# AdamCodd/local-hyperDB

Measured on AMD Instinct MI355X. Metric: queries/sec, N=10M d=384 fp16 top-100 (single-query stream; p50 latency alongside), higher is better.
Workload: dtype f16; 1 GPU; N=10000000 d=384 fp16 Q=1 cosine_similarity top-100, row-sharded x1; rows_per_gpu=10000000, accumulate=f32, exchange=none

## Files before the change

local-hyperdb_amd/csrc/hdb_api.hip:

```cpp
#include "hdb_common.h"
#include "hdb_quant.h"
#include "hdb_ws.h"
#include "hdb_plan.h"
#include "../../include/hyperdb_hip.h"
#include <string>
#include <cmath>
#include <cstring>
#include <cstdio>
#include <algorithm>
#include <vector>
#include <chrono>
#include <atomic>

static thread_local std::string g_err;
static int fail(int code, const std::string& msg) { g_err = msg; return code; }
#define HIP_TRY(expr)                                                                              \
    do {                                                                                           \
        hipError_t e_ = (expr);                                                                    \
        if (e_ != hipSuccess)                                                                      \
            return fail(HDB_ERR_HIP, std::string(#expr) + ": " + hipGetErrorString(e_));           \
    } while (0)
#define LAUNCH_TRY(expr)                                                                           \
    do {                                                                                           \
        int e_ = (expr);                                                                           \
// ... 697 lines not shown
    int rc = quant_ws_lay(ix, w, nq, (nq == 1 && ix->pnib) ? p.pl_cap : 0, mflavour);
    if (rc) return rc;
    const uint32_t pl_cap = p.pl_cap;
    uint32_t* pl_cnt = use_pl ? reinterpret_cast<uint32_t*>(ix->qstat) + 1 : nullptr;
    const size_t crow = (size_t)nq * HDB_CAND_CAP;
    const int nsub = p.nsub;
    rc = quant_query_prep(ix, (const float*)dev_Q, nq, w, mflavour, ix->qstat, nsub ? w.cnt : nullptr, pl_cnt, st);
    if (rc) return rc;
    QuantArgs a; quant_base_args(ix, a, w.qcodes, w.qaux, w.qinv, metric, nq);
    a.ntiles = sp.s_tiles; a.tile_stride = sp.s_stride; a.scores = w.sbuf; a.ld = sp.ld_s;
    a.wmax = w.wmax; a.nsub = nsub; a.thr_out = w.thr;
    LAUNCH_TRY(hdb_launch_quant_scan(&a, 0, (int)ix->opt.max_blocks, st));
    if (!nsub) LAUNCH_TRY(hdb_launch_sample_thr(w.sbuf, sp.s_rows, sp.ld_s, nq, m, w.thr, w.cnt, nullptr, st));
    a.ntiles = (n + 15) / 16; a.tile_stride = 1; a.scores = nullptr; a.ld = 0;
    a.thr = w.thr; a.cnt = w.cnt; a.cand = w.cand; a.cap = HDB_CAND_CAP;
    prof_begin(ix, st);
    if (use_pl) {
        a.pl_nib = ix->pnib; a.pl_bit = ix->pbit; a.pl_rec = ix->prec; a.pl_units = ix->pU;
        a.pl_list = w.pl_list; a.pl_cnt = pl_cnt; a.pl_cap = pl_cap;
        LAUNCH_TRY(hdb_launch_quant_plane_scan(&a, 0, (int)ix->opt.max_blocks, st));
        a.nsub = 0; a.wmax = nullptr;
        LAUNCH_TRY(hdb_launch_quant_scan_one(&a, 1, (int)ix->opt.max_blocks, st));
    } else {
        LAUNCH_TRY(hdb_launch_quant_scan(&a, 1, (int)ix->opt.max_blocks, st));
    }
    prof_end(ix, st);
    if (mflavour) {
        const bool has_bias = ix->bias != nullptr || ix->mask != nullptr;
        LAUNCH_TRY(hdb_launch_quant_cgather(ix->V, ix->d * 2, ix->inv_norm, ix->bias, ix->mask, w.cand, w.cnt, HDB_CAND_CAP, nq, w.G,
                                            metric == HDB_COSINE ? w.ginv : nullptr, has_bias ? w.gbias : nullptr, st));
        ScanArgs s; memset(&s, 0, sizeof(s));
        s.V = w.G; s.n = (int64_t)crow; s.d = ix->d; s.Q = dev_Q; s.metric = metric; s.inv_norm = w.ginv; s.qinv = w.qinv;
        s.bias = has_bias ? w.gbias : nullptr; s.mask = nullptr; s.nq = nq;
        s.tile_stride = 1; s.ntiles = (int64_t)crow / hdb_mfma_tile_rows(ix->dtype, ix->d); s.cap = HDB_CAND_CAP;
        s.scores = w.gsc; s.ld = (int64_t)crow;
        LAUNCH_TRY(hdb_launch_mfma_scan(&s, ix->dtype, 0, nq, w.q16, w.ginv, w.qsq, w.qscl, (int)ix->opt.max_blocks, (int)ix->opt.mfma_variant, st, nullptr));
    } else {
        LAUNCH_TRY(hdb_launch_quant_rescore(ix->V, ix->d, ix->dtype, (const float*)dev_Q, nq, metric, ix->inv_norm, w.qinv, ix->bias, ix->mask,
                                            w.cand, w.cnt, HDB_CAND_CAP, st));
    }
    LAUNCH_TRY(hdb_launch_quant_finalize(w.cand, w.cnt, HDB_CAND_CAP, nq, (uint32_t)k, kk, ix->row_base, dev_idx, dev_score, dev_status, w.qnan,
                                         w.qaux, w.thr, ix->qstat, mflavour ? w.cand : nullptr, w.gsc, (int64_t)crow, st));
    return HDB_OK;
}

// ... 711 lines not shown
```

local-hyperdb_amd/csrc/hdb_launch.h:

```cpp
#pragma once
#include <stddef.h>
#include <stdint.h>

struct ScanArgs;
struct FusedArgs;
struct BatchArgs;
struct BitsArgs;
struct QuantArgs;

#define HDB_ANYD_DECL(name) int name(const ScanArgs* args, int dpad, int mode, int nq_launch, const void* q, const float* sqnorm, \
                                     const float* qsq, const float* qscl, int blocks, void* stream)
#define HDB_GEOM_DECL(name) int name(const ScanArgs* args, int mode, int nq_launch, const void* q16, const float* sqnorm, \
                                     const float* qsq, const float* qscl, int blocks, int variant, void* stream, const BatchArgs* f)

extern "C" {
int hdb_launch_scan(const ScanArgs* args, int dtype, int mode, int nq_launch, int max_blocks, void* stream);
int hdb_launch_rownorm(const void* V, int64_t n, int d, int dtype, float* inv_norm, float* sqnorm, int* nan_flag, void* stream);
int hdb_launch_qprep(const void* Q, int nq, int d, bool f64, float* qinv, float* qsq, int* qnan, void* q16, float* qscl, void* stream);
int hdb_launch_qprep2(const void* Q, int nq, int d, bool f64, float* qinv, float* qsq, int* qnan, void* q16, float* qscl,
                      float* thr_init, uint32_t* cnt_init, uint32_t* qbits, int W, void* stream);
int hdb_launch_signpack(const void* V, int64_t n, int d, int dtype, int64_t row0, uint32_t* bits, void* stream);
int hdb_launch_qsign(const void* Q, int nq, int d, bool f64, int W, uint32_t* qbits, void* stream);
int hdb_launch_hamming(const ScanArgs* args, int mode, int nq_launch, const uint32_t* bits, int64_t npad, int W,
                       const uint32_t* qbits, void* stream);
// ... 69 lines not shown
int hdb_launch_quant_rows(const void* V, int64_t n, int d, int dtype, int P, int8_t* codes, float* aux, int* nan_flag, double gamma,
                          void* stream);
int hdb_launch_quant_gather(const int8_t* codes, const float* aux, const int64_t* rows, int64_t m, int P, int8_t* codes_out,
                            float* aux_out, void* stream);
int hdb_launch_quant_qprep(const float* Q, int nq, int d, int P, int8_t* qcodes, float* qaux, int* stat, uint32_t* pl_cnt, void* stream);
int hdb_launch_quant_qprep_m(const float* Q, int nq, int d, int P, float* qinv, float* qsq, int* qnan, void* q16, float* qscl,
                             int8_t* qcodes, float* qaux, int* stat, uint32_t* cnt_init, uint32_t* pl_cnt, void* stream);
int hdb_launch_quant_plane_rows(const int8_t* codes, const float* aux, int64_t row0, int64_t m, int d, int P, uint8_t* nib, uint32_t* bitw,
                                float* rec, void* stream);
int hdb_launch_quant_plane_scan(const QuantArgs* args, int dbg, int max_blocks, void* stream);
int hdb_launch_quant_scan(const QuantArgs* args, int mode, int max_blocks, void* stream);
int hdb_launch_quant_scan_one(const QuantArgs* args, int mode, int max_blocks, void* stream);
int hdb_launch_quant_rescore(const void* V, int d, int dtype, const float* Q, int nq, int metric, const float* inv_norm,
                             const float* qinv, const float* bias, const uint8_t* mask, unsigned long long* cand,
                             const uint32_t* cnt, uint32_t cap, void* stream);
int hdb_launch_quant_cgather(const void* V, int row_bytes, const float* inv_norm, const float* bias, const uint8_t* mask,
                             const unsigned long long* cand, const uint32_t* cnt, uint32_t cap, int nq, void* G, float* ginv, float* gbias,
                             void* stream);
int hdb_launch_quant_finalize(const unsigned long long* cand, const uint32_t* cnt, uint32_t cap, int nq, uint32_t k, uint32_t kk,
                              int64_t row_base, int64_t* idx_out, float* score_out, int32_t* status, const int* qnan,
                              const float* qaux, const float* thr, int* stat, unsigned long long* cand_rw, const float* sc, int64_t ld,
                              void* stream);

int hdb_launch_qb_scan(const QuantArgs* args, int mode, float* wstat, int64_t wld, int max_blocks, void* stream);
int hdb_launch_qb_thr(const float* vals, int64_t n, int64_t ld, int nq, uint32_t m, float* thr, void* stream);
int hdb_launch_qb_rescore(const void* V, int d, const void* q16, const float* qscl, const float* qinv, const float* inv_norm,
                          const float* bias, const uint8_t* mask, int metric, unsigned long long* cand, const uint32_t* cnt,
                          uint32_t cap, int nq, void* stream);
}
```

local-hyperdb_amd/csrc/hdb_quant.h:

```cpp
#pragma once
#include <stdint.h>

#define HDB_QROW_S 0
#define HDB_QROW_E 1
#define HDB_QROW_T 2
#define HDB_QQ_S 0
#define HDB_QQ_N 1
#define HDB_QQ_D 2
#define HDB_QQ_SQ 3
#define HDB_QQ_BAD 4
#define HDB_QQ_CN 5
#define HDB_QQ_CS 6
#define HDB_QQ_WORDS 8

struct QuantArgs {
    const int8_t* codes;
    int64_t n;
    int32_t d;
    int32_t P;
    const float* aux;
    const float* sqnorm;
    const float* inv_norm;
    const int8_t* qcodes;
    const float* qaux;
    const float* qinv;
    const float* bias;
    const uint8_t* mask;
    int32_t metric;
    int32_t nq;
    float gamma;
    int64_t ntiles;
    int64_t tile_stride;
    float* scores; int64_t ld;
    const float* thr; uint32_t* cnt; unsigned long long* cand; uint32_t cap;
    uint32_t* wmax; int32_t nsub; float* thr_out;
    const uint8_t* pl_nib; const uint32_t* pl_bit; const float* pl_rec; int32_t pl_units;
    uint32_t* pl_list; uint32_t* pl_cnt; uint32_t pl_cap;
    float* dbg;
};
#define HDB_QUANT_NSUB_MAX 4096
```

local-hyperdb_amd/csrc/hdb_quant.hip:

```cpp
#include "hdb_common.h"
#include "hdb_quant.h"
#include "hdb_finalize.h"
#include "../../include/hyperdb_hip.h"

__device__ __forceinline__ float hq_up(double x) {
    x = x * (1.0 + 0x1p-40);
    float f = (float)x;
    if ((double)f < x) f = nextafterf(f, INFINITY);
    return f;
}

__device__ __forceinline__ float hq_f(__half v) { return __half2float(v); }
__device__ __forceinline__ float hq_f(float v) { return v; }

template <typename T> struct HqElem;
template <> struct HqElem<__half> { static constexpr int EPC = 8; };
template <> struct HqElem<float> { static constexpr int EPC = 4; };

__device__ __forceinline__ void hq_unpack(const uint4& raw, float (&x)[8], __half*) {
    const __half2* h = reinterpret_cast<const __half2*>(&raw);
#pragma unroll
    for (int i = 0; i < 4; ++i) { float2 f = __half22float2(h[i]); x[2 * i] = f.x; x[2 * i + 1] = f.y; }
}
__device__ __forceinline__ void hq_unpack(const uint4& raw, float (&x)[4], float*) {
// ... 206 lines not shown
    case 2: return __builtin_amdgcn_update_dpp(0, x, HDB_DPP_XOR2, 0xF, 0xF, false);
    default: return __builtin_amdgcn_update_dpp(0, x, HDB_DPP_XOR1, 0xF, 0xF, false);
    }
}
__device__ __forceinline__ int hq_rows4_sum(int a0, int a1, int a2, int a3, int l16) {
    const bool b3 = (l16 & 8) != 0, b2 = (l16 & 4) != 0;
    const int v01 = (b3 ? a1 : a0) + hq_dpp_i(b3 ? a0 : a1, 0);
    const int v23 = (b3 ? a3 : a2) + hq_dpp_i(b3 ? a2 : a3, 0);
    int w = (b2 ? v23 : v01) + hq_dpp_i(b2 ? v01 : v23, 1);
    w += hq_dpp_i(w, 2);
    w += hq_dpp_i(w, 3);
    return w;
}

template <int NQ>
__device__ __forceinline__ void hq_fold_thr(const QuantArgs& a, float (&q_thr)[NQ]) {
    __shared__ uint32_t s_top[4 * 16];
    __shared__ float s_thr[NQ];
    const int ln = threadIdx.x & 63, wv = threadIdx.x >> 6;
    for (int q = 0; q < NQ; ++q) {
        uint32_t c[HDB_QUANT_NSUB_MAX / 256];
#pragma unroll
        for (int j = 0; j < HDB_QUANT_NSUB_MAX / 256; ++j) {
            const int e = (int)threadIdx.x + 256 * j;
            c[j] = e < a.nsub ? a.wmax[(int64_t)q * a.nsub + e] : 0u;
        }
        for (int r = 0; r < 16; ++r) {
            uint32_t lm = 0u;
#pragma unroll
            for (int j = 0; j < HDB_QUANT_NSUB_MAX / 256; ++j) lm = max(lm, c[j]);
            uint32_t wm = lm;
#pragma unroll
            for (int o = 32; o > 0; o >>= 1) wm = max(wm, (uint32_t)__shfl_xor((int)wm, o, 64));
            const unsigned long long who = __ballot(lm == wm);
            if (ln == (int)__ffsll((long long)who) - 1) {
                bool gone = false;
#pragma unroll
                for (int j = 0; j < HDB_QUANT_NSUB_MAX / 256; ++j)
                    if (!gone && c[j] == wm) { c[j] = 0u; gone = true; }
            }
// ... 9 lines not shown
                for (int o = 32; o > 0; o >>= 1) wm = max(wm, (uint32_t)__shfl_xor((int)wm, o, 64));
                const unsigned long long who = __ballot(v == wm);
                if (ln == (int)__ffsll((long long)who) - 1) v = 0u;
                kth = wm;
            }
            if (ln == 0) {
                const float t = kth == 0u ? -INFINITY : hdb_key2f(kth);
                s_thr[q] = t;
                if (blockIdx.x == 0) a.thr_out[q] = t;
            }
        }
        __syncthreads();
    }
#pragma unroll
    for (int q = 0; q < NQ; ++q) q_thr[q] = s_thr[q];
}

template <int MODE, int NQ, int NJ, bool LIST = false>
__global__ __launch_bounds__(256) void hdb_quant_scan_kernel(QuantArgs a) {
    extern __shared__ __attribute__((aligned(16))) char smem[];
    int4* qs = reinterpret_cast<int4*>(smem);
    __shared__ HqStage stage;
    const int nch = a.P >> 4;
    static_assert(!LIST || (MODE == 1 && NQ == 1), "the list flavour is pass 2 of a one-query call");
    if (MODE == 1 && threadIdx.x < 4) stage.cnt[threadIdx.x] = 0u;
    for (int i = threadIdx.x; i < NQ * nch; i += 256) qs[i] = reinterpret_cast<const int4*>(a.qcodes)[i];
    float q_s[NQ], q_n[NQ], q_d[NQ], q_sq[NQ], q_inv[NQ], q_thr[NQ];
    bool q_bad[NQ];
#pragma unroll
    for (int q = 0; q < NQ; ++q) {
        const float* o = a.qaux + (int64_t)q * HDB_QQ_WORDS;
        q_s[q] = o[HDB_QQ_S]; q_n[q] = o[HDB_QQ_N]; q_d[q] = o[HDB_QQ_D]; q_sq[q] = o[HDB_QQ_SQ]; q_bad[q] = o[HDB_QQ_BAD] != 0.f;
        q_inv[q] = a.metric == HDB_COSINE ? a.qinv[q] : 1.f;
        q_thr[q] = (MODE == 1 && a.nsub == 0) ? a.thr[q] : 0.f;
    }
    __syncthreads();
    if (MODE == 1 && a.nsub > 0) hq_fold_thr<NQ>(a, q_thr);

    const int lane = threadIdx.x & 63, wave = threadIdx.x >> 6;
    const int g = lane >> 4, l16 = lane & 15;
    const int nj = NJ > 0 ? NJ : (nch + 15) >> 4;
    constexpr int G = NJ > 0 ? NJ : 2;
    const float absmin = 0x1p-100f * (float)(a.d + 8);
    const float g2 = 2.f * a.gamma;
    typedef unsigned int u32x4 __attribute__((ext_vector_type(4)));
    uint32_t wbest[NQ];
#pragma unroll
    for (int q = 0; q < NQ; ++q) wbest[q] = 0u;

    int64_t ntiles = a.ntiles;
    uint32_t pl_n = 0u;
    bool pl_list = false;
// ... 2 lines not shown
        pl_list = pl_n <= a.pl_cap;
        if (pl_list) ntiles = ((int64_t)pl_n + 15) >> 4;
        else if (blockIdx.x == 0 && threadIdx.x == 0) atomicAdd(&a.pl_cnt[1], 1u);
    }
    for (int64_t t = (int64_t)blockIdx.x * 4 + wave; t < ntiles; t += (int64_t)gridDim.x * 4) {
        const int64_t r0 = hdb_tile_index(t, a.tile_stride) * 16 + 4 * g;
        int64_t rr[4];
#pragma unroll
        for (int u = 0; u < 4; ++u) {
            rr[u] = r0 + u;
            if (LIST && pl_list) rr[u] = (uint64_t)(r0 + u) < (uint64_t)pl_n ? (int64_t)a.pl_list[r0 + u] : a.n;
        }
        const int8_t* p[4];
#pragma unroll
        for (int u = 0; u < 4; ++u) p[u] = a.codes + min(rr[u], a.n - 1) * (int64_t)a.P;
        int acc[4][NQ];
#pragma unroll
        for (int u = 0; u < 4; ++u)
#pragma unroll
            for (int q = 0; q < NQ; ++q) acc[u][q] = 0;
        for (int j0 = 0; j0 < nj; j0 += G) {
            uint4 raw[G][4];
#pragma unroll
            for (int j = 0; j < G; ++j) {
                const int c = l16 + 16 * (j0 + j);
                const bool live = (j0 + j) < nj && c < nch;
#pragma unroll
                for (int u = 0; u < 4; ++u) {
                    if (live) {
                        const u32x4 v = __builtin_nontemporal_load(reinterpret_cast<const u32x4*>(p[u] + (int64_t)c * 16));
// ... 11 lines not shown
#pragma unroll
                for (int q = 0; q < NQ; ++q) {
                    const int4 qv = qs[q * nch + cc];
#pragma unroll
                    for (int u = 0; u < 4; ++u) {
                        int s = acc[u][q];
                        s = __builtin_amdgcn_sdot4((int)raw[j][u].x, qv.x, s, false);
                        s = __builtin_amdgcn_sdot4((int)raw[j][u].y, qv.y, s, false);
                        s = __builtin_amdgcn_sdot4((int)raw[j][u].z, qv.z, s, false);
                        s = __builtin_amdgcn_sdot4((int)raw[j][u].w, qv.w, s, false);
                        acc[u][q] = s;
                    }
                }
            }
        }
        const int u_own = hdb_owned_row(l16);
        const int64_t row = LIST ? (u_own == 0 ? rr[0] : u_own == 1 ? rr[1] : u_own == 2 ? rr[2] : rr[3]) : r0 + u_own;
        int C[NQ];
#pragma unroll
        for (int q = 0; q < NQ; ++q) C[q] = hq_rows4_sum(acc[0][q], acc[1][q], acc[2][q], acc[3][q], l16);
        if ((l16 & 3) != 0) continue;
        const int64_t out_i = t * 16 + 4 * g + u_own;
        if (row >= a.n) {
            if (MODE == 0 && a.nsub == 0)
#pragma unroll
                for (int q = 0; q < NQ; ++q) a.scores[(int64_t)q * a.ld + out_i] = -INFINITY;
            continue;
        }
        const float s_r = a.aux[3 * row + HDB_QROW_S], e_r = a.aux[3 * row + HDB_QROW_E], t_r = a.aux[3 * row + HDB_QROW_T];
        const bool masked = a.mask && !a.mask[row];
        const float bias = a.bias ? a.bias[row] : 0.f;
        const float invn = a.metric == HDB_COSINE ? a.inv_norm[row] : 1.f;
        const float sqv = a.metric == HDB_EUCLIDEAN ? a.sqnorm[row] : 0.f;
#pragma unroll
        for (int q = 0; q < NQ; ++q) {
            float lo = -INFINITY, hi = -INFINITY;
            if (!q_bad[q] && !masked) {
                const float A = (q_s[q] * s_r) * (float)C[q];
                const float aA = fabsf(A);
                const float B = (q_n[q] * e_r + q_d[q] * t_r) * (1.f + 0x1p-10f) + aA * 0x1p-10f + absmin;
                if (a.metric == HDB_EUCLIDEAN) {
                    const float ctr = sqv + q_sq[q] - 2.f * A;
                    const float err = g2 * sqv + 2.f * B + 0x1p-10f * (sqv + q_sq[q] + 2.f * aA) + absmin;
                    const float elo = fmaxf(ctr - err, 0.f) * (1.f - g2 - 0x1p-10f);
                    const float ehi = (ctr + err) * (1.f + g2 + 0x1p-10f);
                    hi = (float)(1.f / (1.f + sqrt(elo)));
                    lo = (float)(1.f / (1.f + sqrt(ehi)));
                } else {
// ... 5 lines not shown
                hi = hi + fabsf(hi) * 0x1p-20f + 1e-30f;
                if (lo != lo) lo = -INFINITY;
                if (hi != hi) hi = INFINITY;
            }
            if (MODE == 2) {
                a.dbg[row] = hi;
            } else if (MODE == 0) {
                if (a.nsub > 0) wbest[q] = max(wbest[q], hdb_f2key(lo));
                else a.scores[(int64_t)q * a.ld + out_i] = lo;
            } else if (!masked && !q_bad[q] && hi >= q_thr[q]) {
                const unsigned long long ent = hdb_pack(hi, (uint32_t)row);
                const unsigned int lp = atomicAdd(&stage.cnt[q], 1u);
                if (lp < HQ_STAGE_CAP) stage.buf[q][lp] = ent;
                else {
                    const uint32_t pos = atomicAdd(&a.cnt[q * HDB_CNT_STRIDE], 1u);
                    if (pos < a.cap) a.cand[(int64_t)q * a.cap + pos] = ent;
                }
            }
        }
    }
    if (MODE == 0 && a.nsub > 0) {
#pragma unroll
        for (int q = 0; q < NQ; ++q) {
            uint32_t wm = wbest[q];
#pragma unroll
            for (int o = 32; o > 0; o >>= 1) wm = max(wm, (uint32_t)__shfl_xor((int)wm, o, 64));
            if (lane == 0) a.wmax[(int64_t)q * a.nsub + blockIdx.x * 4 + wave] = wm;
        }
    }
    if (MODE == 1) {
        __syncthreads();
        for (int q = 0; q < NQ; ++q) {
            const unsigned int have = min(stage.cnt[q], (unsigned int)HQ_STAGE_CAP);
            if (have == 0u) continue;
            if (threadIdx.x == 0) stage.base = atomicAdd(&a.cnt[q * HDB_CNT_STRIDE], have);
            __syncthreads();
            const unsigned int base = stage.base;
            for (unsigned int e = threadIdx.x; e < have; e += blockDim.x)
                if (base + e < a.cap) a.cand[(int64_t)q * a.cap + base + e] = stage.buf[q][e];
            __syncthreads();
        }
    }
}

__global__ __launch_bounds__(256) void hdb_quant_plane_rows_kernel(const int8_t* codes, const float* aux, int64_t row0, int64_t m, int d, int P,
                                                                   int U, uint8_t* nib, uint32_t* bitw, float* rec) {
    const int lane = threadIdx.x & 63, g = lane >> 4, l16 = lane & 15;
    const int64_t wave = ((int64_t)blockIdx.x * 256 + threadIdx.x) >> 6;
    const int64_t nwaves = ((int64_t)gridDim.x * 256) >> 6;
    for (int64_t base = wave * 4; base < m; base += nwaves * 4) {
        const int64_t r = row0 + base + g;
        const bool valid = base + g < m;
        int ss = 0;
        if (valid && l16 < U) {
// ... 17 lines not shown
                }
            }
            *reinterpret_cast<uint4*>(nib + (r * (int64_t)U + l16) * 16) = make_uint4(nw[0], nw[1], nw[2], nw[3]);
            bitw[r * (int64_t)U + l16] = bw;
        }
#pragma unroll
        for (int o = 8; o > 0; o >>= 1) ss += __shfl_xor(ss, o, 64);
        if (valid && l16 == 0) {
            const float R = sqrtf((float)ss) * (1.f + 0x1p-20f);
            *reinterpret_cast<float4*>(rec + 4 * r) = make_float4(aux[3 * r + HDB_QROW_S], aux[3 * r + HDB_QROW_E], aux[3 * r + HDB_QROW_T], R);
        }
    }
}

#define HQ_PL_STAGE 1024
template <int J, bool DBG>
__global__ __launch_bounds__(256) void hdb_quant_plane_scan_kernel(QuantArgs a) {
    extern __shared__ __attribute__((aligned(16))) char smem[];
    int4* qs = reinterpret_cast<int4*>(smem);
    __shared__ int part[4][2][64 * J];
    __shared__ uint32_t st_buf[HQ_PL_STAGE];
    __shared__ uint32_t st_cnt, st_base;
    const int U = a.pl_units, nch = a.P >> 4;
    if (threadIdx.x == 0) st_cnt = 0u;
    for (int i = threadIdx.x; i < 2 * U; i += 256) qs[i] = i < nch ? reinterpret_cast<const int4*>(a.qcodes)[i] : make_int4(0, 0, 0, 0);
    const float* qo = a.qaux;
    const float q_s = qo[HDB_QQ_S], q_n = qo[HDB_QQ_N], q_d = qo[HDB_QQ_D], q_cn = qo[HDB_QQ_CN];
    const int q_cs = (int)qo[HDB_QQ_CS];
    const bool q_bad = qo[HDB_QQ_BAD] != 0.f;
    const bool cosine = a.metric == HDB_COSINE;
    const float q_inv = cosine ? a.qinv[0] : 1.f;
    float thr1[1] = {(!DBG && a.nsub == 0) ? a.thr[0] : 0.f};
    __syncthreads();
    if (!DBG && a.nsub > 0) hq_fold_thr<1>(a, thr1);
    const float q_thr = thr1[0];

    const int lane = threadIdx.x & 63, wave = threadIdx.x >> 6;
    const int npieces = 16 * U;
    int qw[J][8];
    int prow[J];
#pragma unroll
    for (int j = 0; j < J; ++j) {
        const int f = lane + 64 * j;
        const int unit = f < npieces ? f % U : 0;
        prow[j] = f < npieces ? f / U : 16;
        const int4 x = qs[2 * unit], y = qs[2 * unit + 1];
        qw[j][0] = x.x; qw[j][1] = x.y; qw[j][2] = x.z; qw[j][3] = x.w;
        qw[j][4] = y.x; qw[j][5] = y.y; qw[j][6] = y.z; qw[j][7] = y.w;
    }
    const float absmin = 0x1p-100f * (float)(a.d + 8);
    typedef unsigned int u32x4 __attribute__((ext_vector_type(4)));
    typedef float f32x4 __attribute__((ext_vector_type(4)));
    const int64_t ntiles = a.ntiles;
    const int et = lane >> 4, er = lane & 15;

    for (int64_t t = ((int64_t)blockIdx.x * 4 + wave) * 2; t < ntiles; t += (int64_t)gridDim.x * 8) {
        u32x4 nv[2][J];
        uint32_t bv[2][J];
#pragma unroll
        for (int tt = 0; tt < 2; ++tt) {
            const int64_t rows_left = a.n - (t + tt) * 16;
            const uint8_t* nb = a.pl_nib + (t + tt) * (int64_t)npieces * 16;
            const uint32_t* bb = a.pl_bit + (t + tt) * (int64_t)npieces;
#pragma unroll
            for (int j = 0; j < J; ++j) {
                const int f = lane + 64 * j;
                if ((int64_t)prow[j] < rows_left && prow[j] < 16) {
                    nv[tt][j] = __builtin_nontemporal_load(reinterpret_cast<const u32x4*>(nb + (int64_t)f * 16));
                    bv[tt][j] = __builtin_nontemporal_load(bb + f);
                } else {
                    nv[tt][j] = u32x4{0u, 0u, 0u, 0u};
                    bv[tt][j] = 0u;
                }
            }
        }
        const int64_t row = (t + et) * 16 + er;
        const bool rvalid = lane < 32 && t + et < ntiles && row < a.n;
        f32x4 rc = f32x4{0.f, 0.f, 0.f, 0.f};
        float invn = 1.f, bias = 0.f;
        bool masked = false;
        if (rvalid) {
            rc = __builtin_nontemporal_load(reinterpret_cast<const f32x4*>(a.pl_rec) + row);
            if (cosine) invn = a.inv_norm[row];
            if (a.bias) bias = a.bias[row];
            if (a.mask) masked = !a.mask[row];
        }
        __builtin_amdgcn_sched_barrier(0);
#pragma unroll
        for (int tt = 0; tt < 2; ++tt) {
#pragma unroll
            for (int j = 0; j < J; ++j) {
                const uint32_t bw = bv[tt][j];
                const uint32_t w4[4] = {nv[tt][j].x, nv[tt][j].y, nv[tt][j].z, nv[tt][j].w};
                int s = 0;
#pragma unroll
                for (int i = 0; i < 4; ++i) {
                    const uint32_t lo = ((w4[i] << 1) & 0x1E1E1E1Eu) | ((bw >> (2 * i)) & 0x01010101u);
                    const uint32_t hi = ((w4[i] >> 3) & 0x1E1E1E1Eu) | ((bw >> (2 * i + 1)) & 0x01010101u);
                    s = __builtin_amdgcn_sdot4((int)lo, qw[j][2 * i], s, false);
                    s = __builtin_amdgcn_sdot4((int)hi, qw[j][2 * i + 1], s, false);
                }
                part[wave][tt][lane + 64 * j] = s;
            }
        }
        __builtin_amdgcn_fence(__ATOMIC_RELEASE, "wavefront");
        __builtin_amdgcn_wave_barrier();
        __builtin_amdgcn_fence(__ATOMIC_ACQUIRE, "wavefront");
        int S = 0;
        if (lane < 32)
            for (int i = 0; i < U; ++i) S += part[wave][et][er * U + i];
        __builtin_amdgcn_fence(__ATOMIC_RELEASE, "wavefront");
        __builtin_amdgcn_wave_barrier();
        if (!rvalid) continue;
        float hi5 = -INFINITY;
        const bool dead = masked || q_bad;
        if (!dead) {
            const float fc = (float)(8 * S - 124 * q_cs);
            const float Uf = q_cn * rc.w;
            float ch = fc + Uf, cl = fc - Uf;
            ch = ch + (fabsf(ch) * 0x1p-20f + 1.f);
            cl = cl - (fabsf(cl) * 0x1p-20f + 1.f);
            const float k = q_s * rc.x;
            const float A5 = k * ch, Al = k * cl;
            const float Amax = fmaxf(fabsf(A5), fabsf(Al));
            const float c0 = (q_n * rc.y + q_d * rc.z) * (1.f + 0x1p-10f);
            const float B5 = c0 + fabsf(A5) * 0x1p-10f + absmin;
            const float Bmax = c0 + Amax * 0x1p-10f + absmin;
            const float Mx = Amax + Bmax;
            float X = (A5 + B5) + (Mx * 0x1p-18f + 1e-30f);
            float mM = Mx * (1.f + 0x1p-17f);
// ... 1 lines not shown
            const float Z = mM + fabsf(bias);
            float h = X;
            if (a.bias) h += bias;
            hi5 = h + (Z * 0x1p-18f + 4e-30f);
            if (hi5 != hi5) hi5 = INFINITY;
        }
        if (DBG) {
            a.dbg[row] = hi5;
        } else if (!dead && !(hi5 < q_thr)) {
            const unsigned int lp = atomicAdd(&st_cnt, 1u);
            if (lp < HQ_PL_STAGE) st_buf[lp] = (uint32_t)row;
            else {
                const uint32_t pos = atomicAdd(&a.pl_cnt[0], 1u);
                if (pos < a.pl_cap) a.pl_list[pos] = (uint32_t)row;
            }
        }
    }
    if (!DBG) {
        __syncthreads();
        const unsigned int have = min(st_cnt, (unsigned int)HQ_PL_STAGE);
        if (have != 0u) {
            if (threadIdx.x == 0) st_base = atomicAdd(&a.pl_cnt[0], have);
            __syncthreads();
            const unsigned int base = st_base;
            for (unsigned int e = threadIdx.x; e < have; e += blockDim.x)
                if (base + e < a.pl_cap) a.pl_list[base + e] = st_buf[e];
        }
    }
}

// ... 58 lines not shown
                s = (float)(Acc(1) / (Acc(1) + sqrt(sum)));
            } else if (a.metric == HDB_COSINE) {
                s = (float)sum * a.inv_norm[row] * a.qinv[q];
            } else {
                s = (float)sum;
            }
            if (a.bias) s += a.bias[row];
            const bool masked = a.mask && !a.mask[row];
            if (masked) s = -INFINITY;
            s = hdb_canon(s);
            a.cand[(int64_t)q * a.cap + i] = hdb_pack(s, row);
        }
    }
}

__global__ __launch_bounds__(256) void hdb_quant_cgather_kernel(const char* V, int row_bytes, const float* inv_norm, const float* bias,
                                                                const uint8_t* mask, const unsigned long long* cand, const uint32_t* cnt,
                                                                uint32_t cap, char* G, float* ginv, float* gbias) {
    const int q = blockIdx.y, lane = threadIdx.x & 63, wave = threadIdx.x >> 6;
    const uint32_t total = min(cnt[q * HDB_CNT_STRIDE], cap);
    for (uint32_t i = blockIdx.x * 4 + wave; i < total; i += gridDim.x * 4) {
        const int64_t slot = (int64_t)q * cap + i;
        const uint32_t row = 0xFFFFFFFFu - (uint32_t)(cand[slot] & 0xFFFFFFFFull);
        const char* src = V + (int64_t)row * row_bytes;
        char* dst = G + slot * row_bytes;
        for (int c = lane * 16; c < row_bytes; c += 64 * 16) *reinterpret_cast<uint4*>(dst + c) = *reinterpret_cast<const uint4*>(src + c);
        if (lane == 0) {
            if (ginv) ginv[slot] = inv_norm[row];
            if (gbias) gbias[slot] = mask ? (mask[row] ? (bias ? bias[row] : 0.f) : -INFINITY) : bias[row];
        }
    }
}

__global__ __launch_bounds__(1024) void hdb_quant_finalize_kernel(const unsigned long long* cand, const uint32_t* cnt, uint32_t cap, uint32_t k,
                                                                  uint32_t kk, int64_t row_base, int64_t* idx_out, float* score_out,
                                                                  int32_t* status, const int* qnan, const float* qaux, const float* thr,
                                                                  int* stat, unsigned long long* cand_rw, const float* sc, int64_t ld) {
    extern __shared__ __attribute__((aligned(16))) unsigned long long buf[];
    const int q = blockIdx.x;
    const uint32_t total = cnt[q * HDB_CNT_STRIDE];
    if (sc) {
        const uint32_t nc = min(total, cap);
        for (uint32_t i = threadIdx.x; i < nc; i += blockDim.x) {
            const int64_t slot = (int64_t)q * cap + i;
            const uint32_t row = 0xFFFFFFFFu - (uint32_t)(cand_rw[slot] & 0xFFFFFFFFull);
            cand_rw[slot] = hdb_pack(sc[(int64_t)q * ld + slot], row);
        }
        __threadfence_block();
// ... 25 lines not shown
}

extern "C" int hdb_launch_quant_qprep(const float* Q, int nq, int d, int P, int8_t* qcodes, float* qaux, int* stat, uint32_t* pl_cnt,
                                      void* stream) {
    hipLaunchKernelGGL(hdb_quant_qprep_kernel, dim3(nq), dim3(64), 0, (hipStream_t)stream, Q, nq, d, P, qcodes, qaux, stat, pl_cnt);
    return (int)hipGetLastError();
}

extern "C" int hdb_launch_quant_qprep_m(const float* Q, int nq, int d, int P, float* qinv, float* qsq, int* qnan, void* q16, float* qscl,
                                        int8_t* qcodes, float* qaux, int* stat, uint32_t* cnt_init, uint32_t* pl_cnt, void* stream) {
    hipLaunchKernelGGL(hdb_quant_qprep_m_kernel, dim3(nq), dim3(64), 0, (hipStream_t)stream, Q, nq, d, P, qinv, qsq, qnan, (_Float16*)q16,
                       qscl, qcodes, qaux, stat, cnt_init, pl_cnt);
    return (int)hipGetLastError();
}

extern "C" int hdb_launch_quant_cgather(const void* V, int row_bytes, const float* inv_norm, const float* bias, const uint8_t* mask,
                                        const unsigned long long* cand, const uint32_t* cnt, uint32_t cap, int nq, void* G, float* ginv,
                                        float* gbias, void* stream) {
    if (row_bytes % 16 != 0 || (reinterpret_cast<uintptr_t>(V) & 15) != 0) return (int)hipErrorInvalidValue;
    hipLaunchKernelGGL(hdb_quant_cgather_kernel, dim3(256, nq), dim3(256), 0, (hipStream_t)stream, (const char*)V, row_bytes, inv_norm, bias,
                       mask, cand, cnt, cap, (char*)G, ginv, gbias);
    return (int)hipGetLastError();
}

template <int MODE, int NQ>
static void hq_launch_scan_nq(const QuantArgs& a, int blocks, size_t lds, hipStream_t st) {
    const int nch = a.P >> 4;
    const int nj = (nch + 15) >> 4;
    if (nj == 1) hipLaunchKernelGGL((hdb_quant_scan_kernel<MODE, NQ, 1>), dim3(blocks), dim3(256), lds, st, a);
    else if (nj == 2) hipLaunchKernelGGL((hdb_quant_scan_kernel<MODE, NQ, 2>), dim3(blocks), dim3(256), lds, st, a);
    else if (nj == 3) hipLaunchKernelGGL((hdb_quant_scan_kernel<MODE, NQ, 3>), dim3(blocks), dim3(256), lds, st, a);
    else hipLaunchKernelGGL((hdb_quant_scan_kernel<MODE, NQ, 0>), dim3(blocks), dim3(256), lds, st, a);
}
template <int MODE>
static void hq_launch_scan_mode(const QuantArgs& a, int blocks, size_t lds, hipStream_t st) {
    switch (a.nq) {
    case 1: hq_launch_scan_nq<MODE, 1>(a, blocks, lds, st); break;
    case 2: hq_launch_scan_nq<MODE, 2>(a, blocks, lds, st); break;
    case 3: hq_launch_scan_nq<MODE, 3>(a, blocks, lds, st); break;
    default: hq_launch_scan_nq<MODE, 4>(a, blocks, lds, st); break;
    }
}
extern "C" int hdb_launch_quant_scan(const QuantArgs* args, int mode, int max_blocks, void* stream) {
    const QuantArgs& a = *args;
    if (a.nq < 1 || a.nq > 4 || (a.P & 15) != 0) return (int)hipErrorInvalidValue;
    const size_t lds = (size_t)a.nq * a.P;
    const int blocks = hdb_quant_scan_blocks(a.ntiles, max_blocks);
    if (a.nsub != 0 && (a.nsub > HDB_QUANT_NSUB_MAX || !a.wmax || (mode == 0 ? a.nsub != 4 * blocks : !a.thr_out))) return (int)hipErrorInvalidValue;
    if (mode == 0) hq_launch_scan_mode<0>(a, blocks, lds, (hipStream_t)stream);
    else hq_launch_scan_mode<1>(a, blocks, lds, (hipStream_t)stream);
    return (int)hipGetLastError();
}

extern "C" int hdb_launch_quant_plane_rows(const int8_t* codes, const float* aux, int64_t row0, int64_t m, int d, int P, uint8_t* nib,
                                           uint32_t* bitw, float* rec, void* stream) {
    if (m <= 0) return 0;
    const int U = hdb_quant_plane_units(P);
    if (U > 16 || (P & 15) != 0) return (int)hipErrorInvalidValue;
    hipLaunchKernelGGL(hdb_quant_plane_rows_kernel, dim3(hdb_grid_for(m, 16, 8192)), dim3(256), 0, (hipStream_t)stream, codes, aux, row0, m, d,
                       P, U, nib, bitw, rec);
    return (int)hipGetLastError();
}
extern "C" int hdb_launch_quant_plane_scan(const QuantArgs* args, int dbg, int max_blocks, void* stream) {
    const QuantArgs& a = *args;
    const int U = a.pl_units;
    if (a.nq != 1 || U < 1 || U > 16 || U != hdb_quant_plane_units(a.P) || (a.metric != HDB_DOT && a.metric != HDB_COSINE)) return (int)hipErrorInvalidValue;
    if (!dbg && a.nsub != 0 && (a.nsub > HDB_QUANT_NSUB_MAX || !a.wmax || !a.thr_out)) return (int)hipErrorInvalidValue;
    const size_t lds = (size_t)U * 32;
    const int blocks = hdb_grid_for((a.ntiles + 1) / 2, 4, max_blocks > 0 ? max_blocks : 1024);
    hipStream_t st = (hipStream_t)stream;
    const int J = (U + 3) / 4;
#define HQ_PLANE(J_) do { if (dbg) hipLaunchKernelGGL((hdb_quant_plane_scan_kernel<J_, true>), dim3(blocks), dim3(256), lds, st, a); \
                          else hipLaunchKernelGGL((hdb_quant_plane_scan_kernel<J_, false>), dim3(blocks), dim3(256), lds, st, a); } while (0)
    if (J == 1) HQ_PLANE(1); else if (J == 2) HQ_PLANE(2); else if (J == 3) HQ_PLANE(3); else HQ_PLANE(4);
#undef HQ_PLANE
    return (int)hipGetLastError();
}
extern "C" int hdb_launch_quant_scan_one(const QuantArgs* args, int mode, int max_blocks, void* stream) {
    const QuantArgs& a = *args;
    if (a.nq != 1 || (a.P & 15) != 0 || a.nsub != 0 || (mode != 1 && mode != 2)) return (int)hipErrorInvalidValue;
    const size_t lds = (size_t)a.P;
    const int blocks = hdb_quant_scan_blocks(a.ntiles, max_blocks);
    const int nj = ((a.P >> 4) + 15) >> 4;
    hipStream_t st = (hipStream_t)stream;
#define HQ_ONE(NJ_) do { if (mode == 1) hipLaunchKernelGGL((hdb_quant_scan_kernel<1, 1, NJ_, true>), dim3(blocks), dim3(256), lds, st, a); \
                         else hipLaunchKernelGGL((hdb_quant_scan_kernel<2, 1, NJ_, false>), dim3(blocks), dim3(256), lds, st, a); } while (0)
    if (nj == 1) HQ_ONE(1); else if (nj == 2) HQ_ONE(2); else if (nj == 3) HQ_ONE(3); else HQ_ONE(0);
#undef HQ_ONE
    return (int)hipGetLastError();
}

extern "C" int hdb_launch_quant_rescore(const void* V, int d, int dtype, const float* Q, int nq, int metric, const float* inv_norm,
                                        const float* qinv, const float* bias, const uint8_t* mask, unsigned long long* cand,
                                        const uint32_t* cnt, uint32_t cap, void* stream) {
    hipStream_t st = (hipStream_t)stream;
// ... 34 lines not shown
```

Baseline: 1870 queries/s.

## Fuse candidate row gather into quant scan and software-pipeline plane scan loads

Removes the separate candidate-gather kernel: the quant scan now copies the fp16 row, inverse norm and bias into the gather buffer at the moment a candidate is appended. The plane scan kernel is restructured into a double-buffered loop that issues the next tile's nibble, bit and per-row loads before decoding the current tile. It also overlaps the first loads with the threshold fold and prefetches per-row aux data before the dot loop in the generic scan. The aim is to save a kernel launch plus a second pass over candidates and to hide memory latency, at the cost of more registers and scattered per-candidate copies inside the hot scan.

```diff
diff --git a/local-hyperdb_amd/csrc/hdb_api.hip b/local-hyperdb_amd/csrc/hdb_api.hip
--- a/local-hyperdb_amd/csrc/hdb_api.hip
+++ b/local-hyperdb_amd/csrc/hdb_api.hip
@@ -735,6 +735,11 @@
     if (!nsub) LAUNCH_TRY(hdb_launch_sample_thr(w.sbuf, sp.s_rows, sp.ld_s, nq, m, w.thr, w.cnt, nullptr, st));
     a.ntiles = (n + 15) / 16; a.tile_stride = 1; a.scores = nullptr; a.ld = 0;
     a.thr = w.thr; a.cnt = w.cnt; a.cand = w.cand; a.cap = HDB_CAND_CAP;
+    const bool has_bias = ix->bias != nullptr || ix->mask != nullptr;
+    if (mflavour) {
+        a.V = (const char*)ix->V; a.row_bytes = ix->d * 2; a.G = w.G;
+        a.ginv = metric == HDB_COSINE ? w.ginv : nullptr; a.gbias = has_bias ? w.gbias : nullptr;
+    }
     prof_begin(ix, st);
     if (use_pl) {
         a.pl_nib = ix->pnib; a.pl_bit = ix->pbit; a.pl_rec = ix->prec; a.pl_units = ix->pU;
@@ -747,9 +752,6 @@
     }
     prof_end(ix, st);
     if (mflavour) {
-        const bool has_bias = ix->bias != nullptr || ix->mask != nullptr;
-        LAUNCH_TRY(hdb_launch_quant_cgather(ix->V, ix->d * 2, ix->inv_norm, ix->bias, ix->mask, w.cand, w.cnt, HDB_CAND_CAP, nq, w.G,
-                                            metric == HDB_COSINE ? w.ginv : nullptr, has_bias ? w.gbias : nullptr, st));
         ScanArgs s; memset(&s, 0, sizeof(s));
         s.V = w.G; s.n = (int64_t)crow; s.d = ix->d; s.Q = dev_Q; s.metric = metric; s.inv_norm = w.ginv; s.qinv = w.qinv;
         s.bias = has_bias ? w.gbias : nullptr; s.mask = nullptr; s.nq = nq;
diff --git a/local-hyperdb_amd/csrc/hdb_launch.h b/local-hyperdb_amd/csrc/hdb_launch.h
--- a/local-hyperdb_amd/csrc/hdb_launch.h
+++ b/local-hyperdb_amd/csrc/hdb_launch.h
@@ -107,9 +107,6 @@
 int hdb_launch_quant_rescore(const void* V, int d, int dtype, const float* Q, int nq, int metric, const float* inv_norm,
                              const float* qinv, const float* bias, const uint8_t* mask, unsigned long long* cand,
                              const uint32_t* cnt, uint32_t cap, void* stream);
-int hdb_launch_quant_cgather(const void* V, int row_bytes, const float* inv_norm, const float* bias, const uint8_t* mask,
-                             const unsigned long long* cand, const uint32_t* cnt, uint32_t cap, int nq, void* G, float* ginv, float* gbias,
-                             void* stream);
 int hdb_launch_quant_finalize(const unsigned long long* cand, const uint32_t* cnt, uint32_t cap, int nq, uint32_t k, uint32_t kk,
                               int64_t row_base, int64_t* idx_out, float* score_out, int32_t* status, const int* qnan,
                               const float* qaux, const float* thr, int* stat, unsigned long long* cand_rw, const float* sc, int64_t ld,
diff --git a/local-hyperdb_amd/csrc/hdb_quant.h b/local-hyperdb_amd/csrc/hdb_quant.h
--- a/local-hyperdb_amd/csrc/hdb_quant.h
+++ b/local-hyperdb_amd/csrc/hdb_quant.h
@@ -37,5 +37,6 @@
     const uint8_t* pl_nib; const uint32_t* pl_bit; const float* pl_rec; int32_t pl_units;
     uint32_t* pl_list; uint32_t* pl_cnt; uint32_t pl_cap;
     float* dbg;
+    const char* V; int32_t row_bytes; char* G; float* ginv; float* gbias;
 };
 #define HDB_QUANT_NSUB_MAX 4096
diff --git a/local-hyperdb_amd/csrc/hdb_quant.hip b/local-hyperdb_amd/csrc/hdb_quant.hip
--- a/local-hyperdb_amd/csrc/hdb_quant.hip
+++ b/local-hyperdb_amd/csrc/hdb_quant.hip
@@ -244,16 +244,26 @@
 }
 
 template <int NQ>
-__device__ __forceinline__ void hq_fold_thr(const QuantArgs& a, float (&q_thr)[NQ]) {
+__device__ __forceinline__ void hq_fold_keys(const QuantArgs& a, int q, uint32_t (&c)[HDB_QUANT_NSUB_MAX / 256]) {
+#pragma unroll
+    for (int j = 0; j < HDB_QUANT_NSUB_MAX / 256; ++j) {
+        const int e = (int)threadIdx.x + 256 * j;
+        const uint32_t v = a.wmax[(int64_t)q * a.nsub + min(e, a.nsub - 1)];
+        c[j] = e < a.nsub ? v : 0u;
+    }
+}
+template <int NQ>
+__device__ __forceinline__ void hq_fold_thr(const QuantArgs& a, float (&q_thr)[NQ], const uint32_t (&k0)[HDB_QUANT_NSUB_MAX / 256]) {
     __shared__ uint32_t s_top[4 * 16];
     __shared__ float s_thr[NQ];
     const int ln = threadIdx.x & 63, wv = threadIdx.x >> 6;
     for (int q = 0; q < NQ; ++q) {
         uint32_t c[HDB_QUANT_NSUB_MAX / 256];
-#pragma unroll
-        for (int j = 0; j < HDB_QUANT_NSUB_MAX / 256; ++j) {
-            const int e = (int)threadIdx.x + 256 * j;
-            c[j] = e < a.nsub ? a.wmax[(int64_t)q * a.nsub + e] : 0u;
+        if (q == 0) {
+#pragma unroll
+            for (int j = 0; j < HDB_QUANT_NSUB_MAX / 256; ++j) c[j] = k0[j];
+        } else {
+            hq_fold_keys<NQ>(a, q, c);
         }
         for (int r = 0; r < 16; ++r) {
             uint32_t lm = 0u;
@@ -293,6 +303,16 @@
     }
 #pragma unroll
     for (int q = 0; q < NQ; ++q) q_thr[q] = s_thr[q];
+}
+
+__device__ __forceinline__ void hq_gather_row(const QuantArgs& a, int64_t slot, uint32_t row, int l0, int nl) {
+    const char* src = a.V + (int64_t)row * a.row_bytes;
+    char* dst = a.G + slot * a.row_bytes;
+    for (int c = l0 * 16; c < a.row_bytes; c += nl * 16) *reinterpret_cast<uint4*>(dst + c) = *reinterpret_cast<const uint4*>(src + c);
+    if (l0 == 0) {
+        if (a.ginv) a.ginv[slot] = a.inv_norm[row];
+        if (a.gbias) a.gbias[slot] = a.mask ? (a.mask[row] ? (a.bias ? a.bias[row] : 0.f) : -INFINITY) : a.bias[row];
+    }
 }
 
 template <int MODE, int NQ, int NJ, bool LIST = false>
@@ -314,7 +334,11 @@
         q_thr[q] = (MODE == 1 && a.nsub == 0) ? a.thr[q] : 0.f;
     }
     __syncthreads();
-    if (MODE == 1 && a.nsub > 0) hq_fold_thr<NQ>(a, q_thr);
+    if (MODE == 1 && a.nsub > 0) {
+        uint32_t keys[HDB_QUANT_NSUB_MAX / 256];
+        hq_fold_keys<NQ>(a, 0, keys);
+        hq_fold_thr<NQ>(a, q_thr, keys);
+    }
 
     const int lane = threadIdx.x & 63, wave = threadIdx.x >> 6;
     const int g = lane >> 4, l16 = lane & 15;
@@ -347,6 +371,17 @@
         const int8_t* p[4];
 #pragma unroll
         for (int u = 0; u < 4; ++u) p[u] = a.codes + min(rr[u], a.n - 1) * (int64_t)a.P;
+        const int u_own = hdb_owned_row(l16);
+        const int64_t row = LIST ? (u_own == 0 ? rr[0] : u_own == 1 ? rr[1] : u_own == 2 ? rr[2] : rr[3]) : r0 + u_own;
+        float s_r = 0.f, e_r = 0.f, t_r = 0.f, bias = 0.f, invn = 1.f, sqv = 0.f;
+        bool masked = false;
+        if ((l16 & 3) == 0 && row < a.n) {
+            s_r = a.aux[3 * row + HDB_QROW_S]; e_r = a.aux[3 * row + HDB_QROW_E]; t_r = a.aux[3 * row + HDB_QROW_T];
+            if (a.mask) masked = !a.mask[row];
+            if (a.bias) bias = a.bias[row];
+            if (a.metric == HDB_COSINE) invn = a.inv_norm[row];
+            if (a.metric == HDB_EUCLIDEAN) sqv = a.sqnorm[row];
+        }
         int acc[4][NQ];
 #pragma unroll
         for (int u = 0; u < 4; ++u)
@@ -388,8 +423,6 @@
                 }
             }
         }
-        const int u_own = hdb_owned_row(l16);
-        const int64_t row = LIST ? (u_own == 0 ? rr[0] : u_own == 1 ? rr[1] : u_own == 2 ? rr[2] : rr[3]) : r0 + u_own;
         int C[NQ];
 #pragma unroll
         for (int q = 0; q < NQ; ++q) C[q] = hq_rows4_sum(acc[0][q], acc[1][q], acc[2][q], acc[3][q], l16);
@@ -401,11 +434,6 @@
                 for (int q = 0; q < NQ; ++q) a.scores[(int64_t)q * a.ld + out_i] = -INFINITY;
             continue;
         }
-        const float s_r = a.aux[3 * row + HDB_QROW_S], e_r = a.aux[3 * row + HDB_QROW_E], t_r = a.aux[3 * row + HDB_QROW_T];
-        const bool masked = a.mask && !a.mask[row];
-        const float bias = a.bias ? a.bias[row] : 0.f;
-        const float invn = a.metric == HDB_COSINE ? a.inv_norm[row] : 1.f;
-        const float sqv = a.metric == HDB_EUCLIDEAN ? a.sqnorm[row] : 0.f;
 #pragma unroll
         for (int q = 0; q < NQ; ++q) {
             float lo = -INFINITY, hi = -INFINITY;
@@ -441,7 +469,10 @@
                 if (lp < HQ_STAGE_CAP) stage.buf[q][lp] = ent;
                 else {
                     const uint32_t pos = atomicAdd(&a.cnt[q * HDB_CNT_STRIDE], 1u);
-                    if (pos < a.cap) a.cand[(int64_t)q * a.cap + pos] = ent;
+                    if (pos < a.cap) {
+                        a.cand[(int64_t)q * a.cap + pos] = ent;
+                        if (a.G) hq_gather_row(a, (int64_t)q * a.cap + pos, (uint32_t)row, 0, 1);
+                    }
                 }
             }
         }
@@ -465,6 +496,10 @@
             const unsigned int base = stage.base;
             for (unsigned int e = threadIdx.x; e < have; e += blockDim.x)
                 if (base + e < a.cap) a.cand[(int64_t)q * a.cap + base + e] = stage.buf[q][e];
+            if (a.G)
+                for (unsigned int e = wave; e < have; e += 4)
+                    if (base + e < a.cap)
+                        hq_gather_row(a, (int64_t)q * a.cap + base + e, 0xFFFFFFFFu - (uint32_t)(stage.buf[q][e] & 0xFFFFFFFFull), lane, 64);
             __syncthreads();
         }
     }
@@ -512,8 +547,46 @@
 }
 
 #define HQ_PL_STAGE 1024
+#ifndef HQ_PL_BLOCKS
+#define HQ_PL_BLOCKS 1024
+#endif
+typedef unsigned int hq_u32x4 __attribute__((ext_vector_type(4)));
+typedef float hq_f32x4 __attribute__((ext_vector_type(4)));
+template <int J>
+struct HqPlStep {
+    hq_u32x4 nv[2][J];
+    uint32_t bv[2][J];
+    hq_f32x4 rc;
+    float invn, bias;
+    uint8_t mask;
+};
+template <int J>
+__device__ __forceinline__ void hq_pl_issue(const QuantArgs& a, int64_t t, int lane, int npieces, const int (&prow)[J], bool cosine,
+                                            HqPlStep<J>& s) {
+#pragma unroll
+    for (int tt = 0; tt < 2; ++tt) {
+        const int64_t rows_left = a.n - (t + tt) * 16;
+        const int64_t f0 = (t + tt) * (int64_t)npieces + lane;
+#pragma unroll
+        for (int j = 0; j < J; ++j) {
+            const int64_t f = ((int64_t)prow[j] < rows_left && prow[j] < 16) ? f0 + 64 * j : 0;
+            s.nv[tt][j] = __builtin_nontemporal_load(reinterpret_cast<const hq_u32x4*>(a.pl_nib) + f);
+            s.bv[tt][j] = __builtin_nontemporal_load(a.pl_bit + f);
+        }
+    }
+    const int64_t row = (t + (lane >> 4)) * 16 + (lane & 15);
+    const int64_t rowc = (lane < 32 && row < a.n) ? row : 0;
+    const float* invp = cosine ? a.inv_norm : a.pl_rec;
+    const float* biasp = a.bias ? a.bias : a.pl_rec;
+    const uint8_t* maskp = a.mask ? a.mask : reinterpret_cast<const uint8_t*>(a.pl_rec);
+    s.rc = __builtin_nontemporal_load(reinterpret_cast<const hq_f32x4*>(a.pl_rec) + rowc);
+    s.invn = invp[rowc];
+    s.bias = biasp[rowc];
+    s.mask = maskp[rowc];
+}
+
 template <int J, bool DBG>
-__global__ __launch_bounds__(256) void hdb_quant_plane_scan_kernel(QuantArgs a) {
+__global__ __launch_bounds__(256, 4) void hdb_quant_plane_scan_kernel(QuantArgs a) {
     extern __shared__ __attribute__((aligned(16))) char smem[];
     int4* qs = reinterpret_cast<int4*>(smem);
     __shared__ int part[4][2][64 * J];
@@ -529,76 +602,50 @@
     const bool cosine = a.metric == HDB_COSINE;
     const float q_inv = cosine ? a.qinv[0] : 1.f;
     float thr1[1] = {(!DBG && a.nsub == 0) ? a.thr[0] : 0.f};
-    __syncthreads();
-    if (!DBG && a.nsub > 0) hq_fold_thr<1>(a, thr1);
-    const float q_thr = thr1[0];
+    uint32_t keys[HDB_QUANT_NSUB_MAX / 256] = {};
+    if (!DBG && a.nsub > 0) hq_fold_keys<1>(a, 0, keys);
 
     const int lane = threadIdx.x & 63, wave = threadIdx.x >> 6;
     const int npieces = 16 * U;
-    int qw[J][8];
     int prow[J];
 #pragma unroll
-    for (int j = 0; j < J; ++j) {
-        const int f = lane + 64 * j;
-        const int unit = f < npieces ? f % U : 0;
-        prow[j] = f < npieces ? f / U : 16;
-        const int4 x = qs[2 * unit], y = qs[2 * unit + 1];
-        qw[j][0] = x.x; qw[j][1] = x.y; qw[j][2] = x.z; qw[j][3] = x.w;
-        qw[j][4] = y.x; qw[j][5] = y.y; qw[j][6] = y.z; qw[j][7] = y.w;
-    }
+    for (int j = 0; j < J; ++j) prow[j] = lane + 64 * j < npieces ? (lane + 64 * j) / U : 16;
+    const int64_t ntiles = a.ntiles;
+    const int64_t tstep = (int64_t)gridDim.x * 8;
+    int64_t t = ((int64_t)blockIdx.x * 4 + wave) * 2;
+    HqPlStep<J> s0, s1;
+    hq_pl_issue<J>(a, t, lane, npieces, prow, cosine, s0);
+    __builtin_amdgcn_sched_barrier(0);
+
+    __syncthreads();
+    if (!DBG && a.nsub > 0) hq_fold_thr<1>(a, thr1, keys);
+    const float q_thr = thr1[0];
+    int qoff[J];
+#pragma unroll
+    for (int j = 0; j < J; ++j) qoff[j] = lane + 64 * j < npieces ? 2 * ((lane + 64 * j) % U) : 0;
     const float absmin = 0x1p-100f * (float)(a.d + 8);
-    typedef unsigned int u32x4 __attribute__((ext_vector_type(4)));
-    typedef float f32x4 __attribute__((ext_vector_type(4)));
-    const int64_t ntiles = a.ntiles;
     const int et = lane >> 4, er = lane & 15;
 
-    for (int64_t t = ((int64_t)blockIdx.x * 4 + wave) * 2; t < ntiles; t += (int64_t)gridDim.x * 8) {
-        u32x4 nv[2][J];
-        uint32_t bv[2][J];
-#pragma unroll
-        for (int tt = 0; tt < 2; ++tt) {
-            const int64_t rows_left = a.n - (t + tt) * 16;
-            const uint8_t* nb = a.pl_nib + (t + tt) * (int64_t)npieces * 16;
-            const uint32_t* bb = a.pl_bit + (t + tt) * (int64_t)npieces;
-#pragma unroll
-            for (int j = 0; j < J; ++j) {
-                const int f = lane + 64 * j;
-                if ((int64_t)prow[j] < rows_left && prow[j] < 16) {
-                    nv[tt][j] = __builtin_nontemporal_load(reinterpret_cast<const u32x4*>(nb + (int64_t)f * 16));
-                    bv[tt][j] = __builtin_nontemporal_load(bb + f);
-                } else {
-                    nv[tt][j] = u32x4{0u, 0u, 0u, 0u};
-                    bv[tt][j] = 0u;
-                }
-            }
-        }
-        const int64_t row = (t + et) * 16 + er;
-        const bool rvalid = lane < 32 && t + et < ntiles && row < a.n;
-        f32x4 rc = f32x4{0.f, 0.f, 0.f, 0.f};
-        float invn = 1.f, bias = 0.f;
-        bool masked = false;
-        if (rvalid) {
-            rc = __builtin_nontemporal_load(reinterpret_cast<const f32x4*>(a.pl_rec) + row);
-            if (cosine) invn = a.inv_norm[row];
-            if (a.bias) bias = a.bias[row];
-            if (a.mask) masked = !a.mask[row];
-        }
-        __builtin_amdgcn_sched_barrier(0);
-#pragma unroll
-        for (int tt = 0; tt < 2; ++tt) {
-#pragma unroll
-            for (int j = 0; j < J; ++j) {
-                const uint32_t bw = bv[tt][j];
-                const uint32_t w4[4] = {nv[tt][j].x, nv[tt][j].y, nv[tt][j].z, nv[tt][j].w};
-                int s = 0;
+    auto decode = [&](int64_t tc, const HqPlStep<J>& s) {
+#pragma unroll
+        for (int j = 0; j < J; ++j) {
+            int qo_j = qoff[j];
+            asm volatile("" : "+v"(qo_j));
+            const int4 x = qs[qo_j], y = qs[qo_j + 1];
+            const int qw[8] = {x.x, x.y, x.z, x.w, y.x, y.y, y.z, y.w};
+#pragma unroll
+            for (int tt = 0; tt < 2; ++tt) {
+                const uint32_t bw = s.bv[tt][j];
+                const uint32_t w4[4] = {s.nv[tt][j].x, s.nv[tt][j].y, s.nv[tt][j].z, s.nv[tt][j].w};
+                int sum = 0;
 #pragma unroll
                 for (int i = 0; i < 4; ++i) {
                     const uint32_t lo = ((w4[i] << 1) & 0x1E1E1E1Eu) | ((bw >> (2 * i)) & 0x01010101u);
                     const uint32_t hi = ((w4[i] >> 3) & 0x1E1E1E1Eu) | ((bw >> (2 * i + 1)) & 0x01010101u);
-                    s = __builtin_amdgcn_sdot4((int)lo, qw[j][2 * i], s, false);
-                    s = __builtin_amdgcn_sdot4((int)hi, qw[j][2 * i + 1], s, false);
+                    sum = __builtin_amdgcn_sdot4((int)lo, qw[2 * i], sum, false);
+                    sum = __builtin_amdgcn_sdot4((int)hi, qw[2 * i + 1], sum, false);
                 }
-                part[wave][tt][lane + 64 * j] = s;
+                part[wave][tt][lane + 64 * j] = sum;
             }
         }
         __builtin_amdgcn_fence(__ATOMIC_RELEASE, "wavefront");
@@ -609,9 +656,12 @@
             for (int i = 0; i < U; ++i) S += part[wave][et][er * U + i];
         __builtin_amdgcn_fence(__ATOMIC_RELEASE, "wavefront");
         __builtin_amdgcn_wave_barrier();
-        if (!rvalid) continue;
+        const int64_t row = (tc + et) * 16 + er;
+        if (!(lane < 32 && row < a.n)) return;
+        const hq_f32x4 rc = s.rc;
+        const float invn = cosine ? s.invn : 1.f, bias = a.bias ? s.bias : 0.f;
         float hi5 = -INFINITY;
-        const bool dead = masked || q_bad;
+        const bool dead = (a.mask && !s.mask) || q_bad;
         if (!dead) {
             const float fc = (float)(8 * S - 124 * q_cs);
             const float Uf = q_cn * rc.w;
@@ -643,6 +693,27 @@
                 const uint32_t pos = atomicAdd(&a.pl_cnt[0], 1u);
                 if (pos < a.pl_cap) a.pl_list[pos] = (uint32_t)row;
             }
+        }
+    };
+
+    if constexpr (J <= 3) {
+        while (t < ntiles) {
+            hq_pl_issue<J>(a, t + tstep, lane, npieces, prow, cosine, s1);
+            __builtin_amdgcn_sched_barrier(0);
+            decode(t, s0);
+            t += tstep;
+            if (t >= ntiles) break;
+            hq_pl_issue<J>(a, t + tstep, lane, npieces, prow, cosine, s0);
+            __builtin_amdgcn_sched_barrier(0);
+            decode(t, s1);
+            t += tstep;
+        }
+    } else {
+        while (t < ntiles) {
+            decode(t, s0);
+            t += tstep;
+            hq_pl_issue<J>(a, t, lane, npieces, prow, cosine, s0);
+            __builtin_amdgcn_sched_barrier(0);
         }
     }
     if (!DBG) {
@@ -731,24 +802,6 @@
     }
 }
 
-__global__ __launch_bounds__(256) void hdb_quant_cgather_kernel(const char* V, int row_bytes, const float* inv_norm, const float* bias,
-                                                                const uint8_t* mask, const unsigned long long* cand, const uint32_t* cnt,
-                                                                uint32_t cap, char* G, float* ginv, float* gbias) {
-    const int q = blockIdx.y, lane = threadIdx.x & 63, wave = threadIdx.x >> 6;
-    const uint32_t total = min(cnt[q * HDB_CNT_STRIDE], cap);
-    for (uint32_t i = blockIdx.x * 4 + wave; i < total; i += gridDim.x * 4) {
-        const int64_t slot = (int64_t)q * cap + i;
-        const uint32_t row = 0xFFFFFFFFu - (uint32_t)(cand[slot] & 0xFFFFFFFFull);
-        const char* src = V + (int64_t)row * row_bytes;
-        char* dst = G + slot * row_bytes;
-        for (int c = lane * 16; c < row_bytes; c += 64 * 16) *reinterpret_cast<uint4*>(dst + c) = *reinterpret_cast<const uint4*>(src + c);
-        if (lane == 0) {
-            if (ginv) ginv[slot] = inv_norm[row];
-            if (gbias) gbias[slot] = mask ? (mask[row] ? (bias ? bias[row] : 0.f) : -INFINITY) : bias[row];
-        }
-    }
-}
-
 __global__ __launch_bounds__(1024) void hdb_quant_finalize_kernel(const unsigned long long* cand, const uint32_t* cnt, uint32_t cap, uint32_t k,
                                                                   uint32_t kk, int64_t row_base, int64_t* idx_out, float* score_out,
                                                                   int32_t* status, const int* qnan, const float* qaux, const float* thr,
@@ -804,15 +857,9 @@
     return (int)hipGetLastError();
 }
 
-extern "C" int hdb_launch_quant_cgather(const void* V, int row_bytes, const float* inv_norm, const float* bias, const uint8_t* mask,
-                                        const unsigned long long* cand, const uint32_t* cnt, uint32_t cap, int nq, void* G, float* ginv,
-                                        float* gbias, void* stream) {
-    if (row_bytes % 16 != 0 || (reinterpret_cast<uintptr_t>(V) & 15) != 0) return (int)hipErrorInvalidValue;
-    hipLaunchKernelGGL(hdb_quant_cgather_kernel, dim3(256, nq), dim3(256), 0, (hipStream_t)stream, (const char*)V, row_bytes, inv_norm, bias,
-                       mask, cand, cnt, cap, (char*)G, ginv, gbias);
-    return (int)hipGetLastError();
-}
-
+static bool hq_gather_ok(const QuantArgs& a) {
+    return !a.G || (a.V && a.row_bytes > 0 && a.row_bytes % 16 == 0 && (reinterpret_cast<uintptr_t>(a.V) & 15) == 0);
+}
 template <int MODE, int NQ>
 static void hq_launch_scan_nq(const QuantArgs& a, int blocks, size_t lds, hipStream_t st) {
     const int nch = a.P >> 4;
@@ -833,7 +880,7 @@
 }
 extern "C" int hdb_launch_quant_scan(const QuantArgs* args, int mode, int max_blocks, void* stream) {
     const QuantArgs& a = *args;
-    if (a.nq < 1 || a.nq > 4 || (a.P & 15) != 0) return (int)hipErrorInvalidValue;
+    if (a.nq < 1 || a.nq > 4 || (a.P & 15) != 0 || !hq_gather_ok(a)) return (int)hipErrorInvalidValue;
     const size_t lds = (size_t)a.nq * a.P;
     const int blocks = hdb_quant_scan_blocks(a.ntiles, max_blocks);
     if (a.nsub != 0 && (a.nsub > HDB_QUANT_NSUB_MAX || !a.wmax || (mode == 0 ? a.nsub != 4 * blocks : !a.thr_out))) return (int)hipErrorInvalidValue;
@@ -857,7 +904,7 @@
     if (a.nq != 1 || U < 1 || U > 16 || U != hdb_quant_plane_units(a.P) || (a.metric != HDB_DOT && a.metric != HDB_COSINE)) return (int)hipErrorInvalidValue;
     if (!dbg && a.nsub != 0 && (a.nsub > HDB_QUANT_NSUB_MAX || !a.wmax || !a.thr_out)) return (int)hipErrorInvalidValue;
     const size_t lds = (size_t)U * 32;
-    const int blocks = hdb_grid_for((a.ntiles + 1) / 2, 4, max_blocks > 0 ? max_blocks : 1024);
+    const int blocks = hdb_grid_for((a.ntiles + 1) / 2, 4, max_blocks > 0 ? max_blocks : HQ_PL_BLOCKS);
     hipStream_t st = (hipStream_t)stream;
     const int J = (U + 3) / 4;
 #define HQ_PLANE(J_) do { if (dbg) hipLaunchKernelGGL((hdb_quant_plane_scan_kernel<J_, true>), dim3(blocks), dim3(256), lds, st, a); \
@@ -868,7 +915,7 @@
 }
 extern "C" int hdb_launch_quant_scan_one(const QuantArgs* args, int mode, int max_blocks, void* stream) {
     const QuantArgs& a = *args;
-    if (a.nq != 1 || (a.P & 15) != 0 || a.nsub != 0 || (mode != 1 && mode != 2)) return (int)hipErrorInvalidValue;
+    if (a.nq != 1 || (a.P & 15) != 0 || a.nsub != 0 || (mode != 1 && mode != 2) || !hq_gather_ok(a)) return (int)hipErrorInvalidValue;
     const size_t lds = (size_t)a.P;
     const int blocks = hdb_quant_scan_blocks(a.ntiles, max_blocks);
     const int nj = ((a.P >> 4) + 15) >> 4;
```

After: 1836 queries/s. 1.8% lower.
